# jwscook/DistributedHouseholderQR.jl

Hardware: AMD Instinct MI355X
Metric: QR GFLOP/s (F = 2mn^2 - 2/3 n^3), ||A-QR||/||A|| alongside (higher is better)
Workload: dtype f64; 1 GPU; 32768x32768 Float64 dense QR, blocked nb=128 (BASELINE configs[2]); m=32768, n=32768, nb=128, parallelism=single GPU

## Files before the change

### distributedhouseholderqr.jl_amd/csrc/dhqr_api.hip

```cpp
#include <chrono>
#include <mutex>

#include "dhqr_internal.h"
#include "dhqr_complex.h"
#include "dhqr_gemm.h"
#include "dhqr_pack.h"
#include "dhqr_panel.h"
#include "dhqr_recon.h"
#include "dhqr_solve.h"
#include "dhqr_qtb.h"
#include "dhqr_small.h"
#include "dhqr_tsqr.h"

static thread_local char g_err[512] = "";
int32_t set_err(int32_t code, const char *fmt, ...) {
  va_list ap;
  va_start(ap, fmt);
  vsnprintf(g_err, sizeof(g_err), fmt, ap);
  va_end(ap);
  return code;
}
int32_t ensure(dhqr_ctx *c, Buf &b, size_t need) {
  if (need <= b.cap) return DHQR_OK;
  if (b.p) {
// ... 478 lines not shown
    double *out = (l == lv.L()) ? Rroot : bufs[l & 1];
    hipLaunchKernelGGL(k_tsqr_node, dim3((unsigned)lv.cnt[l]), dim3(1024), 0, c->stream, (const double *)nullptr, (int64_t)0,
                       (int64_t)0, in, (int)lv.cnt[l - 1], out, Ybase ? Ybase + (size_t)lv.yoff[l] * 2 * TSQR_NN : nullptr,
                       (int64_t)0);
    in = out;
  }
  LAUNCHCHECK();
  return DHQR_OK;
}
static int32_t tsqr_pairs_down(dhqr_ctx *c, int64_t count, const double *Ybase, const double *Croot, double *ping,
                               double *pong, const double **Cleaf) {
  if (count <= 1) {
    if (Croot == nullptr) {
      hipLaunchKernelGGL(k_tsqr_identity, dim3((unsigned)(TSQR_NN / 256)), dim3(256), 0, c->stream, ping);
      LAUNCHCHECK();
      *Cleaf = ping;
    } else {
      *Cleaf = Croot;
    }
    return DHQR_OK;
  }
  const TsqrLevels lv(count);
  const double *in = Croot;
  double *bufs[2] = {ping, pong};
  for (int l = lv.L(); l >= 1; --l) {
    double *out = bufs[l & 1];
    hipLaunchKernelGGL(k_tsqr_apply, dim3((unsigned)lv.cnt[l]), dim3(1024), 0, c->stream, in,
                       Ybase + (size_t)lv.yoff[l] * 2 * TSQR_NN, (int64_t)0, 0, (int)lv.cnt[l - 1], out, (double *)nullptr,
                       (int64_t)0);
    in = out;
  }
  LAUNCHCHECK();
  *Cleaf = in;
  return DHQR_OK;
}
struct TsqrLocal {
  int64_t rows = 0, nleaf = 0, ldy = 0;
  double *R0 = nullptr, *ping = nullptr, *pong = nullptr, *Yl = nullptr, *Yp = nullptr;
  static size_t elems(int64_t rows) {
    const size_t nl = (size_t)std::max<int64_t>(1, (rows + TSQR_LEAF - 1) / TSQR_LEAF);
    return (3 * nl + 2) * TSQR_NN + nl * 2 * TSQR_NN + (size_t)TsqrLevels::node_blocks((int64_t)nl) * 2 * TSQR_NN;
  }
  void place(double *base, int64_t rows_) {
    rows = rows_;
    nleaf = std::max<int64_t>(1, (rows + TSQR_LEAF - 1) / TSQR_LEAF);
    ldy = nleaf * TSQR_LEAF;
    R0 = base;
    ping = R0 + (size_t)nleaf * TSQR_NN;
    pong = ping + (size_t)(nleaf + 1) * TSQR_NN;
    Yl = pong + (size_t)(nleaf + 1) * TSQR_NN;
    Yp = Yl + (size_t)nleaf * 2 * TSQR_NN;
  }
};
static int32_t tsqr_local_up(dhqr_ctx *c, const TsqrLocal &t, const double *P, int64_t ldp, double *Rroot, bool keep) {
  if (t.rows <= 0) {
    HIPCHECK(hipMemsetAsync(Rroot, 0, TSQR_NN * sizeof(double), c->stream));
    if (keep) HIPCHECK(hipMemsetAsync(t.Yl, 0, (size_t)t.nleaf * 2 * TSQR_NN * sizeof(double), c->stream));
    return DHQR_OK;
  }
  double *lvl0 = (t.nleaf == 1) ? Rroot : t.R0;
  hipLaunchKernelGGL(k_tsqr_node, dim3((unsigned)t.nleaf), dim3(1024), 0, c->stream, P, ldp, t.rows, (const double *)nullptr, 0,
                     lvl0, keep ? t.Yl : (double *)nullptr, t.ldy);
  LAUNCHCHECK();
  if (t.nleaf == 1) return DHQR_OK;
  return tsqr_pairs_up(c, lvl0, t.nleaf, Rroot, keep ? t.Yp : nullptr, t.ping, t.pong);
}
static int32_t tsqr_local_down(dhqr_ctx *c, const TsqrLocal &t, const double *Croot) {
  if (t.rows <= 0) return DHQR_OK;
  const double *Cleaf = nullptr;
  CHECK(tsqr_pairs_down(c, t.nleaf, t.Yp, Croot, t.ping, t.pong, &Cleaf));
  hipLaunchKernelGGL(k_tsqr_apply, dim3((unsigned)t.nleaf), dim3(1024), 0, c->stream, Cleaf, (const double *)t.Yl, t.ldy, 1, 0,
                     (double *)nullptr, t.Yl, t.ldy);
  LAUNCHCHECK();
  return DHQR_OK;
}
static int32_t tsqr_local_r(dhqr_ctx *c, const double *P, int64_t ldp, int64_t rows, double *Rout) {
  CHECK(ensure(c, c->tsq, TsqrLocal::elems(rows)));
  TsqrLocal t;
  t.place(c->tsq.p, rows);
  return tsqr_local_up(c, t, P, ldp, Rout, false);
}

static inline size_t panel_rbuf_elems() { return 6 * (size_t)DHQR_NBV * DHQR_NBV + 1024; }
static inline double *panel_rbuf(dhqr_ctx *c, int panel_idx) { return c->rbuf.p + (size_t)(panel_idx & 1) * panel_rbuf_elems(); }
static int32_t panel_commit_enqueue(dhqr_ctx *c, hipStream_t stream, double *P, int64_t rows, int64_t ldp, double *alpha,
                                    const PanelBuf &pb, int panel_idx, int part = 0) {
  const size_t NN = (size_t)DHQR_NBV * DHQR_NBV;
  const double *Rref = panel_rbuf(c, panel_idx) + 3 * NN, *altmp = panel_rbuf(c, panel_idx) + 6 * NN;
  if (part == 1) {
    hipLaunchKernelGGL(k_commit_alpha, dim3(1), dim3(DHQR_NBV), 0, stream, altmp, (int)DHQR_NBV, (double *)nullptr, pb.alpha,
                       (const int *)c->dstat, panel_idx);
  } else {
    dim3 grid((unsigned)std::min<int64_t>((rows + 255) / 256, 64), DHQR_NBV);
    hipLaunchKernelGGL(k_commit_panel, grid, dim3(256), 0, stream, P, ldp, rows, (const double *)pb.V, pb.ldv, Rref, altmp, alpha,
                       part == 2 ? (double *)nullptr : pb.alpha, (const int *)c->dstat, panel_idx);
  }
  LAUNCHCHECK();
  return DHQR_OK;
}
static int32_t panel_fast_enqueue(dhqr_ctx *c, double *P, int64_t rows, int64_t ldp, double *alpha, const PanelBuf &pb,
                                  int passes, int panel_idx, hipEvent_t ev_v = nullptr, hipEvent_t ev_t = nullptr) {
  const int64_t ldv = pb.ldv;
  const size_t NN = (size_t)DHQR_NBV * DHQR_NBV;
  CHECK(ensure(c, c->rbuf, 2 * panel_rbuf_elems()));
  if (passes == 2) CHECK(ensure(c, c->vts, (size_t)panel_elems(rows)));
  if (passes == 3) CHECK(ensure(c, c->tsq, TsqrLocal::elems(rows)));
  CHECK(ensure(c, c->sfull, NN));
  if (c->ev_commit[panel_idx & 1]) HIPCHECK(hipStreamWaitEvent(c->stream, c->ev_commit[panel_idx & 1], 0));
  double *R1 = panel_rbuf(c, panel_idx), *negR1inv = R1 + NN, *Rf = R1 + 2 * NN, *Rref = R1 + 3 * NN, *negMinv = R1 + 4 * NN;
  double *G = R1 + 5 * NN, *altmp = R1 + 6 * NN;
  int *bflag = c->dstat + 1;
  CHECK(prof_begin(c, CAT_PANEL));
  const bool was = c->profiling;
  c->profiling = false;
  auto body = [&]() -> int32_t {
    const double *X = P;
    int64_t ldx = ldp;
    if (passes == 3) {
      TsqrLocal t;
      t.place(c->tsq.p, rows);
      CHECK(tsqr_local_up(c, t, P, ldp, Rf, true));
      CHECK(tsqr_local_down(c, t, nullptr));
      hipLaunchKernelGGL(k_tsqr_identity, dim3((unsigned)(NN / 256)), dim3(256), 0, c->stream, R1);
      X = t.Yl;
      ldx = t.ldy;
      launch_recon_top(c, X, ldx, R1, G, Rref, negMinv);
      hipLaunchKernelGGL(k_tsqr_sign_cols, dim3((unsigned)(NN / 256)), dim3(256), 0, c->stream, negMinv, (const double *)Rf);
    } else if (passes == 2) {
      CHECK(gram128(c, P, ldp, rows, G));
      double *Q1 = c->vts.p;
      const int64_t ldq = panel_ldv(rows);
      launch_chol_inv(c, G, nullptr, R1, negR1inv, bflag);
      CHECK(mul128(c, P, ldp, rows, negR1inv, Q1, ldq));
      CHECK(gram128(c, Q1, ldq, rows, G));
      launch_chol_inv(c, G, R1, Rf, nullptr, bflag);
      launch_recon_top(c, P, ldp, Rf, altmp, Rref, negMinv);
    } else {
      CHECK(gram128(c, P, ldp, rows, G));
      hipLaunchKernelGGL((k_panel_top<false>), dim3(1), dim3(1024), 0, c->stream, (const double *)G, (const double *)P, ldp, altmp,
                         Rref, negMinv, bflag);
    }
    if (c->fuse_fix) {
      CHECK(mul128(c, X, ldx, rows, negMinv, pb.V, ldv, passes == 3 ? G : altmp));
    } else {
      CHECK(mul128(c, X, ldx, rows, negMinv, pb.V, ldv));
      hipLaunchKernelGGL(k_recon_fix, dim3(NN / 256), dim3(256), 0, c->stream, pb.V, ldv,
                         (const double *)(passes == 3 ? G : altmp), (const double *)negMinv);
    }
    if (ev_v) HIPCHECK(hipEventRecord(ev_v, c->stream));
    if (passes == 3)
      hipLaunchKernelGGL(k_tsqr_final_r, dim3(NN / 256), dim3(256), 0, c->stream, (const double *)Rf, (const double *)G, Rref,
                         altmp);
    CHECK(gram128(c, pb.V, ldv, rows, c->sfull.p));
    hipLaunchKernelGGL(k_build_t, dim3(1), dim3(1024), 0, c->stream, (const double *)c->sfull.p, (int)DHQR_NBV, pb.T, pb.Tt,
                       c->recon_tol, c->dstat, panel_idx, pb.alpha + DHQR_NBV, c->tt_keep);
    if (ev_t) HIPCHECK(hipEventRecord(ev_t, c->stream));
    else CHECK(panel_commit_enqueue(c, c->stream, P, rows, ldp, alpha, pb, panel_idx));
    LAUNCHCHECK();
    return DHQR_OK;
  };
  const int32_t rc = body();
  c->profiling = was;
  CHECK(rc);
  if (c->profiling)
    for (int64_t j = 0; j + 1 < DHQR_NBV; ++j) c->st.bytes_panel += 16.0 * (double)(rows - j) * (double)(DHQR_NBV - j - 1);
  CHECK(prof_end(c));
  return DHQR_OK;
}
static inline bool panel_fast_eligible(dhqr_ctx *c, int64_t rows, int64_t w) {
  return c->panel_impl == 3 && w == DHQR_NBV && rows >= 2 * DHQR_NBV;
}

static int32_t factor_panel_sync(dhqr_ctx *c, double *P, int64_t rows, int64_t w, int64_t ldp, double *alpha,
                                 const PanelBuf &pb) {
  if (panel_fast_eligible(c, rows, w)) {
    const int last_rung = std::max(c->cholqr_passes, c->tsqr_rung == 1 ? 3 : 2);
    for (int passes = c->cholqr_passes; passes <= last_rung; ++passes) {
      CHECK(status_reset(c));
      CHECK(panel_fast_enqueue(c, P, rows, ldp, alpha, pb, passes, 0));
      int failed = 0;
      CHECK(status_read(c, &failed));
      if (failed == INT_MAX) {
        c->n_fast++;
        if (passes == 3) c->n_tsqr++;
        return DHQR_OK;
      }
    }
    CHECK(status_reset(c));
    c->n_fallback++;
  }
  if (c->panel_impl >= 2 && !(c->partial_unblocked && rows > 256 && rows <= c->partial_unblocked_max_rows))
    return factor_panel_v2(c, P, rows, w, ldp, alpha, pb);
  CHECK(factor_unblocked_cols(c, P, rows, w, ldp, alpha, CAT_PANEL));
  return panel_pack_and_t(c, P, rows, w, ldp, alpha, pb);
}

static int32_t comm_allreduce_sum(dhqr_comm *cm, double *dbuf, int64_t count, hipStream_t stream);

static inline int64_t nn_row_chunks(const dhqr_ctx *c, int64_t row_tiles) {
  if (c->nn_split <= 1 || c->cur_ws != 0) return 1;
  return std::max<int64_t>(1, std::min<int64_t>(c->nn_split, row_tiles / c->nn_chunk_tiles));
}

static int32_t narrow_vtc(dhqr_ctx *c, const double *Vp, int64_t ldv, int64_t rows, const double *C, int64_t ldc,
                          int64_t ncols, bool vec, Buf &part, double *Y) {
  const int64_t ntiles = (ncols + 127) / 128, ld2 = 2 * DHQR_NBV, wstride = ld2 * ncols;
  int64_t nsplit, rps;
  pick_split(rows, 2 * ntiles, 512, 256 / ntiles, &nsplit, &rps, 512, 64);
  CHECK(ensure(c, part, (size_t)nsplit * (size_t)wstride));
  const dim3 grid((unsigned)ntiles, (unsigned)nsplit, 2);
  if (vec)
    hipLaunchKernelGGL((k_gemm_tn<2, 1, 128>), grid, dim3(256), 0, c->stream, Vp, ldv, C, ldc, 1, (int64_t)0, rows, ncols, rps, part.p,
                       ld2, wstride);
  else
    hipLaunchKernelGGL((k_gemm_tn<1, 1, 128>), grid, dim3(256), 0, c->stream, Vp, ldv, C, ldc, 1, (int64_t)0, rows, ncols, rps, part.p,
                       ld2, wstride);
  hipLaunchKernelGGL(k_reduce_splits, dim3((unsigned)((wstride + 63) / 64)), dim3(256), 0, c->stream, (const double *)part.p, (int)nsplit,
                     wstride, wstride, Y);
  return DHQR_OK;
}

static int32_t pair_vtc(dhqr_ctx *c, const double *Vp, int64_t ldv, int64_t rows, const double *C, int64_t ldc,
                        int64_t ncols, bool vec, double *Y) {
  const int64_t ntiles = (ncols + 127) / 128;
  if (ntiles <= 2) return narrow_vtc(c, Vp, ldv, rows, C, ldc, ncols, vec, c->ws[c->cur_ws].w1, Y);
  int64_t nsplit, rps;
  const int64_t slots = wide_slots(c, ncols);
  pick_split(rows, ntiles, slots, ntiles <= 2 ? 256 : 64, &nsplit, &rps, slots, ntiles <= 2 ? 64 : 128);
  if (ntiles >= c->tn_model_min_tiles) {
    const int64_t cap = std::min<int64_t>(64, std::max<int64_t>(1, rows / 512));
    double best = 1e300;
    int64_t bns = 1;
    for (int64_t ns = 1; ns <= cap; ++ns) {
      if (ns > 1 && ntiles * ns > 3072) break;
      int64_t r = (rows + ns - 1) / ns;
      r = (r + G_KT - 1) / G_KT * G_KT;
      const int64_t rounds = (ntiles * ns + slots - 1) / slots;
      const double est = (double)rounds * (double)r + (double)ns * (double)ncols * 4.79e-3 + 40.0 * (double)rounds;
      if (est < best) { best = est; bns = ns; }
    }
    int64_t r = (rows + bns - 1) / bns;
    r = (r + G_KT - 1) / G_KT * G_KT;
    rps = r;
    nsplit = std::max<int64_t>(1, (rows + r - 1) / r);
  }
  dhqr_ctx::WS &ws = c->ws[c->cur_ws];
  const int64_t ld2 = 2 * DHQR_NBV, wstride = ld2 * ncols;
  if (ntiles >= c->tn_model_min_tiles && ntiles <= 1024 && rows >= 1024) {
    const int64_t FU = 128, S = (rows + FU - 1) / FU, U = ntiles * S;
    const int64_t G = std::min<int64_t>(U, slots), q = (U + G - 1) / G, Gq = (U + q - 1) / q;
    int R = c->tn2_rgroups;
    if (R == 0) R = rows >= c->tn2_rg8_rows ? 8 : rows >= c->tn2_rg4_rows ? 4 : rows >= c->tn2_rg2_rows ? 2 : 1;
    if (G < 64 || S < 4 * R) R = 1;
    if (R > 1) {
      int P = 0;
      for (int g = 0; g < R; ++g) P = std::max(P, tn2_sk_pieces(tn2_sk_group_of(g, R, G, S, ntiles, q)));
      CHECK(ensure(c, ws.w1, (size_t)R * (size_t)P * (size_t)wstride));
      if (vec)
        hipLaunchKernelGGL((k_gemm_tn2<2, true>), dim3((unsigned)G), dim3(512), 0, c->stream, Vp, ldv, C, ldc, rows, ncols, FU, ws.w1.p, wstride, q, R, P);
      else
        hipLaunchKernelGGL((k_gemm_tn2<1, true>), dim3((unsigned)G), dim3(512), 0, c->stream, Vp, ldv, C, ldc, rows, ncols, FU, ws.w1.p, wstride, q, R, P);
      hipLaunchKernelGGL(k_reduce_pieces, dim3((unsigned)((wstride + 255) / 256)), dim3(256), 0, c->stream, (const double *)ws.w1.p, S, q,
                         wstride, wstride, Y, R, P, G, ntiles);
      return DHQR_OK;
    }
    const int64_t pieces = (q >= S) ? 2 : (S + q - 1) / q + 1;
    CHECK(ensure(c, ws.w1, (size_t)pieces * (size_t)wstride));
    if (vec)
      hipLaunchKernelGGL((k_gemm_tn2<2, true>), dim3((unsigned)Gq), dim3(512), 0, c->stream, Vp, ldv, C, ldc, rows, ncols, FU, ws.w1.p, wstride, q, 1, 0);
    else
      hipLaunchKernelGGL((k_gemm_tn2<1, true>), dim3((unsigned)Gq), dim3(512), 0, c->stream, Vp, ldv, C, ldc, rows, ncols, FU, ws.w1.p, wstride, q, 1, 0);
    hipLaunchKernelGGL(k_reduce_pieces, dim3((unsigned)((wstride + 255) / 256)), dim3(256), 0, c->stream, (const double *)ws.w1.p, S, q,
                       wstride, wstride, Y, 1, 0, Gq, ntiles);
    return DHQR_OK;
  }
  CHECK(ensure(c, ws.w1, (size_t)nsplit * (size_t)wstride));
  const dim3 gtn((unsigned)std::min<int64_t>(ntiles * nsplit, slots)), gred((unsigned)((wstride + 63) / 64));
  if (vec)
    hipLaunchKernelGGL((k_gemm_tn2<2>), gtn, dim3(512), 0, c->stream, Vp, ldv, C, ldc, rows, ncols, rps, ws.w1.p, wstride, (int64_t)0, 1, 0);
  else
    hipLaunchKernelGGL((k_gemm_tn2<1>), gtn, dim3(512), 0, c->stream, Vp, ldv, C, ldc, rows, ncols, rps, ws.w1.p, wstride, (int64_t)0, 1, 0);
  hipLaunchKernelGGL(k_reduce_splits, gred, dim3(256), 0, c->stream, (const double *)ws.w1.p, (int)nsplit, wstride, wstride, Y);
  return DHQR_OK;
}

static int32_t pair_tw(dhqr_ctx *c, double *Y, const double *Ta, const double *Tb, const double *Sba, double *W,
                       int64_t ldw, int64_t ncols) {
  const int64_t ntiles = (ncols + 127) / 128, ld2 = 2 * DHQR_NBV;
  double *Ya = Y, *Yb = Y + DHQR_NBV;
  if (ntiles <= 2) {
    const int64_t NN_ = (int64_t)DHQR_NBV * DHQR_NBV;
    hipLaunchKernelGGL((k_tw_fused<true>), dim3((unsigned)((ncols + 3) / 4)), dim3(256), 0, c->stream, (const double *)Y, ncols,
                       Ta + NN_, Tb + NN_, Sba, W, ldw);
    return DHQR_OK;
  }
  hipLaunchKernelGGL((k_gemm_tn<2, 1, 128>), dim3((unsigned)ntiles, 1), dim3(256), 0, c->stream, Ta, (int64_t)DHQR_NBV,
                     (const double *)Ya, ld2, 1, (int64_t)0, (int64_t)DHQR_NBV, ncols, (int64_t)DHQR_NBV, W, ldw, (int64_t)0);
  launch_nn_sub<128>(c, true, dim3(1, (unsigned)ntiles), Sba, (int64_t)DHQR_NBV, (const double *)W, ldw, Yb, ld2,
                     (int64_t)DHQR_NBV, ncols, 0, false);
  hipLaunchKernelGGL((k_gemm_tn<2, 1, 128>), dim3((unsigned)ntiles, 1), dim3(256), 0, c->stream, Tb, (int64_t)DHQR_NBV,
                     (const double *)Yb, ld2, 1, (int64_t)0, (int64_t)DHQR_NBV, ncols, (int64_t)DHQR_NBV, W + DHQR_NBV, ldw,
                     (int64_t)0);
  return DHQR_OK;
}

static int32_t pair_apply(dhqr_ctx *c, const double *Vp, int64_t ldv, int64_t rows, const double *Ta,
                          const double *Tb, const double *Sba, double *C, int64_t ncols, int64_t ldc,
                          dhqr_comm *ar = nullptr, int64_t rows_b_in = -1) {
// ... 225 lines not shown
  for (int64_t j = 0; j < n; ++j) memcpy(dst + j * ldd, src + j * lds, (size_t)m * sizeof(double));
}

struct DeviceGuard {
  int prev = -1;
  ~DeviceGuard() {
    if (prev >= 0) (void)hipSetDevice(prev);
  }
};
static int32_t enter_ctx(dhqr_ctx *c, DeviceGuard &g) {
  if (!c) return set_err(DHQR_EINVAL, "null context");
  int cur = -1;
  HIPCHECK(hipGetDevice(&cur));
  if (cur != c->device) {
    HIPCHECK(hipSetDevice(c->device));
    g.prev = cur;
  }
  return DHQR_OK;
}
#define ENTER(c_)   \
  DeviceGuard dg_; \
  CHECK(enter_ctx(c_, dg_))
static inline bool no_columns(int64_t m, int64_t n) { return n == 0 && m >= 0; }

static int32_t check_mat(const void *A, int64_t m, int64_t n, int64_t lda, bool need_tall) {
  if (!A) return set_err(DHQR_EINVAL, "null matrix pointer");
  if (m <= 0 || n <= 0) return set_err(DHQR_EINVAL, "m and n must be positive (m=%lld n=%lld)", (long long)m, (long long)n);
  if (need_tall && m < n) return set_err(DHQR_EINVAL, "m >= n required (m=%lld n=%lld)", (long long)m, (long long)n);
  if (lda < m) return set_err(DHQR_EINVAL, "leading dimension %lld < m=%lld", (long long)lda, (long long)m);
  if (lda > (int64_t)0xFFFFFFFFLL / 128)
    return set_err(DHQR_EINVAL, "leading dimension %lld too large (128 * ld must stay below 2^32 elements)", (long long)lda);
  return DHQR_OK;
}

static int32_t apply_q_impl(dhqr_ctx *c, const double *dA, int64_t m, int64_t n, int64_t lda,
                            const double *dalpha, double *dB, int64_t nrhs, int64_t ldb, int trans,
                            bool triangular) {
  const int64_t npan = (n + DHQR_NBV - 1) / DHQR_NBV;
  CHECK(ensure(c, c->vt, (size_t)panel_elems(m)));
  for (int64_t q = 0; q < npan; ++q) {
    const int64_t k = trans ? q : npan - 1 - q;
    const int64_t c0 = k * DHQR_NBV, w = std::min<int64_t>(DHQR_NBV, n - c0), rows = m - c0;
    const double *P = dA + c0 + c0 * lda;
    const PanelBuf pb = vt_view(c->vt.p, rows);
    CHECK(panel_pack_and_t(c, P, rows, w, lda, dalpha ? dalpha + c0 : nullptr, pb));
    if (triangular) {
      if (nrhs - c0 > 0) CHECK(panel_apply(c, pb, rows, dB + c0 + c0 * ldb, nrhs - c0, ldb, trans));
    } else {
      CHECK(panel_apply(c, pb, rows, dB + c0, nrhs, ldb, trans));
    }
  }
  return DHQR_OK;
}

extern "C" {

int32_t dhqr_version(void) { return DHQR_VERSION; }
const char *dhqr_last_error(void) { return g_err; }

int32_t dhqr_device_count(int32_t *count) {
  if (!count) return set_err(DHQR_EINVAL, "null count");
  int n = 0;
  hipError_t e = hipGetDeviceCount(&n);
  if (e != hipSuccess) {
    *count = 0;
    return set_err(DHQR_ENODEVICE, "hipGetDeviceCount: %s", hipGetErrorString(e));
  }
  *count = n;
  return DHQR_OK;
}

int32_t dhqr_create(dhqr_ctx **out, int32_t device) {
  if (!out) return set_err(DHQR_EINVAL, "null ctx out-pointer");
  *out = nullptr;
  int n = 0;
  hipError_t e = hipGetDeviceCount(&n);
  if (e != hipSuccess || n <= 0)
    return set_err(DHQR_ENODEVICE, "no HIP device visible (%s); libdhqr has no CPU fallback",
                   e != hipSuccess ? hipGetErrorString(e) : "count = 0");
  if (device < 0 || device >= n) return set_err(DHQR_EINVAL, "device %d out of range [0,%d)", device, n);
  HIPCHECK(hipSetDevice(device));
  hipDeviceProp_t prop;
  HIPCHECK(hipGetDeviceProperties(&prop, device));
  if (strncmp(prop.gcnArchName, "gfx950", 6) != 0)
    return set_err(DHQR_ENODEVICE, "device %d is %s; this library is built for gfx950 only", device,
                   prop.gcnArchName);
  dhqr_ctx *c = new dhqr_ctx();
  c->device = device;
  c->coop = prop.cooperativeLaunch != 0;
  g_live_ctx[device & 63].fetch_add(1);
  memset(&c->st, 0, sizeof(c->st));
  auto init = [&]() -> int32_t {
    HIPCHECK(hipStreamCreateWithFlags(&c->own, hipStreamNonBlocking));
    c->stream = c->own;
    {
      int lo = 0, hi = 0;
      HIPCHECK(hipDeviceGetStreamPriorityRange(&lo, &hi));
      HIPCHECK(hipStreamCreateWithPriority(&c->hi, hipStreamNonBlocking, hi));
      if (const char *e = getenv("DHQR_LANE_SIDE")) c->lane_side = atoi(e) != 0;
      c->hi_priority = hi;
    }
    if (const char *e = getenv("DHQR_LOOKAHEAD")) c->lookahead = atoi(e) != 0;
    {
      int ncu = 0;
      if (hipDeviceGetAttribute(&ncu, hipDeviceAttributeMultiprocessorCount, device) == hipSuccess && ncu > 0) {
        c->rankk_wgs = ncu;
        c->ncu = ncu;
      }
    }
    if (const char *e = getenv("DHQR_SPARE_CUS")) {
      c->spare_cus = std::max(0, std::min(c->ncu - 8, atoi(e)));
      c->spare_cus_set = true;
    }
    if (const char *e = getenv("DHQR_QUAD")) c->quad = atoi(e) != 0;
    if (const char *e = getenv("DHQR_QUAD_MIN_COLS")) c->quad_min_cols = std::max<int64_t>(0, atoll(e));
    { long long v; if (tune_get("rankk_wgs", &v)) c->rankk_wgs = std::max(2, (int)v); }
    if (const char *e = getenv("DHQR_RANKK")) c->rankk = c->rankk_tall = c->rankk_xtall = std::min(5, std::max(1, atoi(e)));
    if (const char *e = getenv("DHQR_RANKK_MAX")) c->rankk_max = std::min(DHQR_RK_KMAX, std::max(1, atoi(e)));
    { long long v; if (tune_get("rankk_max_min_cols", &v)) c->rankk_max_min_cols = std::max(0, (int)v); }
    { long long v; if (tune_get("nn_chunk_tiles", &v)) c->nn_chunk_tiles = std::max(1, (int)v); }
    if (const char *e = getenv("DHQR_NN_SPLIT")) c->nn_split = std::min(16, std::max(1, atoi(e)));
    if (const char *e = getenv("DHQR_RANKK_PIPE")) c->rankk_pipe = std::min(2, std::max(0, atoi(e)));
    { long long v; if (tune_get("tn_min_tiles", &v)) c->tn_model_min_tiles = (int)v; }
    { long long v; if (tune_get("small_flags", &v)) c->small_flags = v != 0; }
    { long long v; if (tune_get("short_panel_small", &v)) c->short_panel_small = v != 0; }
    { long long v; if (tune_get("partial_unblocked", &v)) c->partial_unblocked = v != 0; }
    { long long v; if (tune_get("partial_unblocked_max_rows", &v)) c->partial_unblocked_max_rows = v; }
    { long long v; if (tune_get("small_spin_limit", &v)) c->small_spin_limit = (int)v; }
    { long long v; if (tune_get("tn2_rgroups", &v)) c->tn2_rgroups = (int)v; }
    { long long v; if (tune_get("tn2_rg8_rows", &v)) c->tn2_rg8_rows = v; }
    { long long v; if (tune_get("tn2_rg4_rows", &v)) c->tn2_rg4_rows = v; }
    { long long v; if (tune_get("tn2_rg2_rows", &v)) c->tn2_rg2_rows = v; }
    { long long v; if (tune_get("tn_spare", &v)) c->tn_spare = std::max(0, std::min((c->ncu - 8) / 2, (int)v)); }
    { long long v; if (tune_get("tn_spare_cols", &v)) c->tn_spare_cols = v; }
    if (const char *e = getenv("DHQR_PAIR")) c->pair = atoi(e) != 0;
    if (const char *e = getenv("DHQR_PAIR_MIN_N")) c->pair_min_n = atoll(e);
    HIPCHECK(hipHostMalloc((void **)&c->hflag, 4 * sizeof(int), hipHostMallocDefault));
    HIPCHECK(hipMalloc((void **)&c->dstat, 16 * sizeof(int)));
    HIPCHECK(hipMalloc((void **)&c->zflags, DHQR_PIPE_INTS * sizeof(int)));
    HIPCHECK(hipMemsetAsync(c->zflags, 0, DHQR_PIPE_INTS * sizeof(int), c->stream));
    {
      int limit = DHQR_PIPE_SPIN_LIMIT;
      { long long v; if (tune_get("spin_limit", &v)) limit = std::max(1, (int)v); }
      HIPCHECK(hipMemcpyAsync(c->zflags + DHQR_PIPE_LIMIT_OFFSET, &limit, sizeof(int), hipMemcpyHostToDevice, c->stream));
      HIPCHECK(hipStreamSynchronize(c->stream));
    }
    if (const char *e = getenv("DHQR_SMALL")) c->small_route = atoi(e) != 0;
    if (const char *e = getenv("DHQR_ZPIPE")) c->zpipe = atoi(e) != 0;
    if (const char *e = getenv("DHQR_SOLVE_PIPE")) c->solve_pipe = std::max(0, std::min(3, atoi(e)));
    if (const char *e = getenv("DHQR_KEEP_T")) c->keep_t = atoi(e) != 0;
    { long long v; if (tune_get("qtb_vec", &v)) c->qtb_vec = (int)v; }
    { long long v; if (tune_get("gram_strips", &v)) c->gram_strips = v != 0; }
    { long long v; if (tune_get("fuse_fix", &v)) c->fuse_fix = v != 0; }
    { long long v; if (tune_get("commit_off", &v)) c->commit_off = (int)v; }
    hipLaunchKernelGGL(k_set_status, dim3(1), dim3(64), 0, c->stream, c->dstat, INT_MAX);
    LAUNCHCHECK();
    HIPCHECK(hipStreamSynchronize(c->stream));
    return DHQR_OK;
  };
  const int32_t rc_init = init();
  if (rc_init != DHQR_OK) {
    (void)dhqr_destroy(c);
    return rc_init;
  }
  if (const char *e = getenv("DHQR_CHOLQR_PASSES")) c->cholqr_passes = atoi(e) == 2 ? 2 : 1;
  if (const char *e = getenv("DHQR_TSQR")) {
    if (atoi(e) != 0) c->cholqr_passes = 3;
  }
  if (const char *e = getenv("DHQR_TSQR_RUNG")) c->tsqr_rung = atoi(e) != 0 ? 1 : 0;
  if (const char *e = getenv("DHQR_PANEL")) {
    const int v = atoi(e);
    if (v >= 1 && v <= 3) c->panel_impl = v;
  }
  *out = c;
  return DHQR_OK;
}

int32_t dhqr_destroy(dhqr_ctx *c) {
  if (!c) return DHQR_OK;
  g_live_ctx[c->device & 63].fetch_sub(1);
  (void)hipSetDevice(c->device);
  (void)hipStreamSynchronize(c->stream);
  (void)hipDeviceSynchronize();
  cs_state_free(c);
  rs_state_free(c);
  if (c->hio) {
    hio_free(*c->hio);
    delete c->hio;
    c->hio = nullptr;
  }
  Buf *bufs[] = {&c->vbuf, &c->vt, &c->vts, &c->ws[0].w1, &c->ws[0].w1r, &c->ws[0].w2, &c->ws[1].w1,
                 &c->ws[1].w1r, &c->ws[1].w2, &c->ws[2].w1, &c->ws[2].w1r, &c->ws[2].w2, &c->spart, &c->spart2, &c->sfull, &c->scratch, &c->pbuf, &c->rbuf, &c->tsq, &c->zsolve_lo, &c->host_mat, &c->sv_T, &c->sv_S, &c->sv_part, &c->sv_small, &c->tc_T, &c->tc_alpha, &c->small_dev, &c->sv_bkp};
  for (Buf *b : bufs)
    if (b->p) (void)hipFree(b->p);
  for (auto &e : c->evs) {
    (void)hipEventDestroy(e.a);
    (void)hipEventDestroy(e.b);
  }
  if (c->hflag) (void)hipHostFree(c->hflag);
  if (c->small_pin) (void)hipHostFree(c->small_pin);
  if (c->dstat) (void)hipFree(c->dstat);
  if (c->zflags) (void)hipFree(c->zflags);
  for (hipEvent_t e : c->zev)
    if (e) (void)hipEventDestroy(e);
  if (c->hi) (void)hipStreamDestroy(c->hi);
  if (c->hi2) (void)hipStreamDestroy(c->hi2);
  if (c->cstream) (void)hipStreamDestroy(c->cstream);
  for (hipEvent_t e : c->ev_commit)
    if (e) (void)hipEventDestroy(e);
  if (c->own) (void)hipStreamDestroy(c->own);
  delete c;
  return DHQR_OK;
}

int32_t dhqr_set_stream(dhqr_ctx *c, void *s) {
  ENTER(c);
  c->stream = (hipStream_t)s;
  return DHQR_OK;
}
int32_t dhqr_use_own_stream(dhqr_ctx *c) {
  ENTER(c);
  c->stream = c->own;
  return DHQR_OK;
}
static int32_t pipe_error_report(dhqr_ctx *c, int e) {
  HIPCHECK(hipMemsetAsync(c->zflags + DHQR_PIPE_ERR_OFFSET, 0, sizeof(int), c->stream));
  HIPCHECK(hipStreamSynchronize(c->stream));
  return set_err(DHQR_EHIP, "an inter-workgroup pipeline (k_zpanel_pipe / rankk_lead_pipe / k_backsub_pipe, launch %d) gave up "
                 "waiting for a lower-indexed workgroup: the results of that call are invalid; DHQR_ZPIPE=0 / DHQR_RANKK_PIPE=0 / "
                 "DHQR_SOLVE_PIPE=0 select the kernels without inter-workgroup waits", e);
}
static int32_t pipe_error_check(dhqr_ctx *c) {
  if (!c->zflags) return DHQR_OK;
  int e = 0;
  HIPCHECK(hipMemcpy(&e, c->zflags + DHQR_PIPE_ERR_OFFSET, sizeof(int), hipMemcpyDeviceToHost));
  if (e == 0) return DHQR_OK;
  if (e == 0x7ffffffe && c->retry.valid) {
    const dhqr_ctx::SolveRetry r = c->retry;
    c->retry.valid = false;
    HIPCHECK(hipMemsetAsync(c->zflags + DHQR_PIPE_ERR_OFFSET, 0, sizeof(int), c->stream));
    HIPCHECK(hipMemcpyAsync(r.b, c->sv_bkp.p, (size_t)r.m * sizeof(double), hipMemcpyDeviceToDevice, c->stream));
    const bool was = c->profiling;
    c->profiling = false;
    const int32_t rc = solve_pipelined(c, r.A, r.m, r.n, r.lda, r.alpha, r.b, false);
    c->profiling = was;
    CHECK(rc);
    HIPCHECK(hipStreamSynchronize(c->stream));
    c->n_solve_retry++;
    HIPCHECK(hipMemcpy(&e, c->zflags + DHQR_PIPE_ERR_OFFSET, sizeof(int), hipMemcpyDeviceToHost));
    if (e == 0) return DHQR_OK;
  }
  return pipe_error_report(c, e);
}

int32_t dhqr_synchronize(dhqr_ctx *c) {
  ENTER(c);
  HIPCHECK(hipStreamSynchronize(c->stream));
  return pipe_error_check(c);
}
int32_t dhqr_trim(dhqr_ctx *c) {
  ENTER(c);
  HIPCHECK(hipStreamSynchronize(c->stream));
  HIPCHECK(hipDeviceSynchronize());
  Buf *bs[] = {&c->host_mat, &c->sv_T, &c->sv_S, &c->sv_part, &c->sv_small, &c->tc_T, &c->tc_alpha, &c->vts, &c->tsq, &c->zsolve_lo,
               &c->small_dev, &c->sv_bkp};
  c->retry.valid = false;
  if (c->small_pin) {
    (void)hipHostFree(c->small_pin);
    c->small_pin = nullptr;
    c->small_pin_cap = 0;
  }
  for (Buf *b : bs)
    if (b->p) {
      (void)hipFree(b->p);
      b->p = nullptr;
      b->cap = 0;
    }
  c->tc_valid = false;
  c->sv_units_dev = nullptr;
  if (c->cs)
    for (Buf &b : c->cs->gbuf)
      if (b.p) {
        (void)hipFree(b.p);
        b.p = nullptr;
        b.cap = 0;
      }
  if (c->hio) {
    hio_free(*c->hio);
    delete c->hio;
    c->hio = nullptr;
  }
  return pipe_error_check(c);
}
int32_t dhqr_set_profiling(dhqr_ctx *c, int32_t on) {
  ENTER(c);
  if (c->profiling && !on) CHECK(prof_resolve(c));
  c->profiling = on != 0;
  return DHQR_OK;
}
int32_t dhqr_reset_stats(dhqr_ctx *c) {
  ENTER(c);
  HIPCHECK(hipStreamSynchronize(c->stream));
  c->ev_used = 0;
  memset(&c->st, 0, sizeof(c->st));
  c->n_fast = c->n_fallback = 0;
  c->n_tsqr = 0;
// ... 1853 lines not shown
```

### distributedhouseholderqr.jl_amd/csrc/dhqr_internal.h

```cpp
#pragma once
#include <hip/hip_runtime.h>

#include <algorithm>
#include <atomic>
#include <climits>
#include <chrono>
#include <cmath>
#include <cstdarg>
#include <cstdio>
#include <cstring>
#include <vector>

#include "../../include/dhqr.h"
#include "dhqr_common.h"

int32_t set_err(int32_t code, const char *fmt, ...);
#define HIPCHECK(expr)                                                                        \
  do {                                                                                        \
    hipError_t e_ = (expr);                                                                   \
    if (e_ != hipSuccess)                                                                     \
      return set_err(DHQR_EHIP, "%s failed: %s (%s:%d)", #expr, hipGetErrorString(e_),        \
                     __FILE__, __LINE__);                                                     \
  } while (0)
#define CHECK(expr)                  \
  do {                               \
    int32_t rc_ = (expr);            \
    if (rc_ != DHQR_OK) return rc_;  \
  } while (0)
#define LAUNCHCHECK() HIPCHECK(hipGetLastError())

enum { CAT_PANEL = 0, CAT_TBUILD, CAT_VTA, CAT_TW, CAT_AVW, CAT_RANK1, CAT_SOLVE, CAT_N };

struct Buf {
  double *p = nullptr;
  size_t cap = 0;
};

struct dhqr_ctx {
  int device = 0;
  hipStream_t own = nullptr, stream = nullptr;
  bool profiling = false;
  hipStream_t hi = nullptr;
  hipStream_t hi2 = nullptr;
  int lane_side = 1;
  int hi_priority = 0;
  int tn_spare = 32;
  int64_t tn_spare_cols = 16384;
  int tn_model_min_tiles = 32;
  int rankk_wgs = 256;
  int rankk = 5;
  int nn_chunk_tiles = 48;
  int nn_split = 4;
  int rankk_pipe = 1;
  int rankk_max_min_cols = 4096;
  int rankk_unfit = 0;
  int rankk_max = 8;
  int rankk_xtall = 5;
  int rankk_tall = 5;
  int ncu = 256;
  int spare_cus = 0;
  bool spare_cus_set = false;
  int quad = 1;
  int64_t quad_min_cols = 10240;
  struct WS { Buf w1, w1r, w2; } ws[3];
  int cur_ws = 0;
  bool lookahead = true;
  Buf vbuf, vt, vts, spart, spart2, sfull, scratch, pbuf;
  Buf zsolve_lo;
  Buf sv_T, sv_S, sv_part, sv_small;
  std::vector<int> sv_units;
  int64_t sv_m = -1, sv_n = -1, sv_rps = 0;
  const int *sv_units_dev = nullptr;
  Buf tc_T, tc_alpha;
  double *tt_keep = nullptr, *tc_base = nullptr;
  const double *tc_A = nullptr;
  int64_t tc_m = 0, tc_n = 0, tc_lda = 0;
  bool tc_valid = false;
  int keep_t = 1;
  int solve_pipe = 1;
  int qtb_vec = -1;
  struct SolveRetry {
    bool valid = false;
    const double *A = nullptr, *alpha = nullptr;
    double *b = nullptr;
    int64_t m = 0, n = 0, lda = 0;
  } retry;
  Buf sv_bkp;
  int64_t n_solve_retry = 0;
  int gram_strips = 1;
  int small_spin_limit = 1 << 20;
  int partial_unblocked = 1;
  int64_t partial_unblocked_max_rows = 4608;
  int short_panel_small = 1;
  int small_flags = 1;
  int tn2_rgroups = 1;
  int64_t tn2_rg8_rows = 20480, tn2_rg4_rows = 10240, tn2_rg2_rows = 5120;
  int fuse_fix = 1;
  int commit_off = -1;
  hipStream_t cstream = nullptr;
  hipEvent_t ev_commit[2] = {nullptr, nullptr};
  int small_route = 1;
  double *small_pin = nullptr;
  size_t small_pin_cap = 0;
  Buf small_dev;
  unsigned long long small_epoch = 0;
  bool coop = false;
  Buf host_mat;
  int pair = 1;
  int64_t pair_min_n = 4096;
  int panel_impl = 3;
  int zpipe = 1;
  hipEvent_t zev[5] = {nullptr, nullptr, nullptr, nullptr, nullptr};
  int *zflags = nullptr;
  int zepoch = 0;
  int *hflag = nullptr;
  int *dstat = nullptr;
  int epoch = -1;
  Buf rbuf;
  Buf tsq;
  int tsqr_rung = -1;
  int n_tsqr = 0;
  int64_t n_fast = 0, n_fallback = 0;
  int cholqr_passes = 1;
  double recon_tol = 2e-12;
  int ib = 64;
  struct CsState *cs = nullptr;
  struct RsState *rs = nullptr;
  int32_t (*panel_hook)(void *, int64_t, hipEvent_t) = nullptr;
  void *panel_hook_arg = nullptr;
  struct HostIo *hio = nullptr;
  int64_t n_resume = 0;
  struct Ev { hipEvent_t a, b; int cat; int start_from = -1; };
  std::vector<Ev> evs;
  size_t ev_used = 0;
  dhqr_stats st;
};


int32_t ensure(dhqr_ctx *c, Buf &b, size_t need);
bool tune_get(const char *key, long long *out);
static inline bool aligned16(const void *p) { return (((uintptr_t)p) & 15) == 0; }
int32_t prof_begin(dhqr_ctx *c, int cat);
int32_t prof_end(dhqr_ctx *c);
int32_t prof_switch(dhqr_ctx *c, int cat);
#define DHQR_RK_KMAX 8
int32_t factor_unblocked_cols(dhqr_ctx *c, double *P, int64_t rows, int64_t ncols, int64_t ldp, double *alpha, int cat);
```

### distributedhouseholderqr.jl_amd/csrc/dhqr_recon.h

```cpp
#pragma once
#include "dhqr_common.h"

#define RC_N 128

__device__ __forceinline__ void rc_upper_inverse_regs(const double (&r)[4][4], double (&x)[4][4],
                                                       double *dinv, double *rowbuf2, double *colbuf2) {
  const int t = threadIdx.x, ti = t >> 5, tk = t & 31;
  double acc[4][4];
#pragma unroll
  for (int a = 0; a < 4; ++a) {
    if (ti == tk) dinv[ti + 32 * a] = 1.0 / r[a][a];
#pragma unroll
    for (int b = 0; b < 4; ++b) { acc[a][b] = 0.0; x[a][b] = 0.0; }
  }
  __syncthreads();
#pragma unroll
  for (int la = 3; la >= 0; --la)
    for (int lm = 31; lm >= 0; --lm) {
      const int l = la * 32 + lm;
      double *rowbuf = rowbuf2 + (l & 1) * RC_N, *colbuf = colbuf2 + (l & 1) * RC_N;
      if (ti == lm) {
        const double di = dinv[l];
#pragma unroll
        for (int b = 0; b < 4; ++b) {
// ... 332 lines not shown
#pragma unroll
  for (int x = 0; x < 4; ++x)
#pragma unroll
    for (int y = 0; y < 4; ++y) negMinv[(ti + 32 * x) + (tk + 32 * y) * RC_N] = mm[x][y];
  __syncthreads();
  double x12[4];
  rc_upper_inverse_blocked(negMinv, RC_N, false, L, x12);
  __syncthreads();
  rc5_emit(L, x12, [&](int i, int k, double v) { negMinv[i + k * RC_N] = -v; });
}

__device__ unsigned long long g_top_phase[8];
template <bool TIME = false>
__device__ __forceinline__ void rc_chol_replay_invert(double (&g)[4][4], double (&a)[4][4], double *rbuf, double *wrow,
                                                      double *vcol, rc5_lds &L, double *__restrict__ alpha,
                                                      double *__restrict__ Rref, double *__restrict__ negMinv,
                                                      int *__restrict__ flag) {
  const int t = threadIdx.x, ti = t >> 5, tk = t & 31, lane = t & 63;
  double *qu = &L.T1[0][0];
#pragma unroll
  for (int ja = 0; ja < 4; ++ja)
    for (int jm = 0; jm < 32; ++jm) {
      const int j = ja * 32 + jm;
      const int src = (lane & 32) + jm;
      long long tq0 = 0, tq1 = 0, tq2 = 0, tq3 = 0;
      if constexpr (TIME) tq0 = clock64();
      double d = __shfl(g[ja][ja], src, 64);
      const double ajj = __shfl(a[ja][ja], src, 64);
      if constexpr (TIME) {
        asm volatile("" : "+v"(d));
        tq1 = clock64();
      }
      double *rb = rbuf + (j & 1) * RC_N, *wr = wrow + (j & 1) * RC_N, *vc = vcol + (j & 1) * RC_N;
      if (ti == jm) {
        if (!(d > 0.0)) {
          if (tk == 0) flag[0] = 1;
          d = 1.0;
        }
        double r, rinv;
        dhqr_sqrt_rsqrt(d, r, rinv);
        const double al = r * dhqr_alphafactor(ajj);
        const double u = dhqr_rcp(ajj - al);
        if (tk == 0) {
          qu[j] = r * (r + fabs(ajj));
          qu[RC_N + j] = u;
        }
        const double sg = (al == 0.0) ? 0.0 : (al < 0.0 ? -1.0 : 1.0);
#pragma unroll
        for (int y = 0; y < 4; ++y) {
          const int k = tk + 32 * y;
          const double x = (k == j) ? r : g[ja][y] * rinv;
          g[ja][y] = x;
          rb[k] = (k > j) ? x : 0.0;
          const double rr = sg * x;
          const double dl = (k > j) ? (a[ja][y] - rr) : 0.0;
          wr[k] = dl * u;
          negMinv[j + k * RC_N] = dl;
          Rref[j + k * RC_N] = (k > j) ? rr : 0.0;
        }
        if (tk == 0) alpha[j] = al;
      }
      if (tk == jm) {
#pragma unroll
        for (int x = 0; x < 4; ++x) {
          const int i = ti + 32 * x;
          vc[i] = (i > j) ? a[x][ja] : 0.0;
        }
      }
      if constexpr (TIME) tq2 = clock64();
      __syncthreads();
      if constexpr (TIME) tq3 = clock64();
#pragma unroll
      for (int x = 0; x < 4; ++x) {
        if (x < ja) continue;
        const double ri = rb[ti + 32 * x], vi = vc[ti + 32 * x];
#pragma unroll
        for (int y = 0; y < 4; ++y) {
          if (y < ja) continue;
          const double rk = rb[tk + 32 * y];
          if (y >= x) g[x][y] = fma(-ri, rk, g[x][y]);
          a[x][y] = fma(-vi, wr[tk + 32 * y], a[x][y]);
        }
      }
      if constexpr (TIME) {
        asm volatile("" : "+v"(a[3][3]), "+v"(g[3][3]));
        const long long tq4 = clock64();
        if (t == 0) {
          g_top_phase[0] += (unsigned long long)(tq1 - tq0);
          g_top_phase[1] += (unsigned long long)(tq2 - tq1);
          g_top_phase[2] += (unsigned long long)(tq3 - tq2);
          g_top_phase[3] += (unsigned long long)(tq4 - tq3);
          g_top_phase[5] += 1ull;
        }
      }
    }
  long long tinv = 0;
  if constexpr (TIME) tinv = clock64();
  __syncthreads();
  if (t < RC_N) {
    const double sq = sqrt(qu[t]);
    qu[t] = sq * qu[RC_N + t];
    qu[RC_N + t] = sq;
  }
  __syncthreads();
  double x12[4];
  rc_upper_inverse_blocked(negMinv, RC_N, false, L, x12, qu);
  __syncthreads();
  rc5_emit(L, x12, [&](int i, int k, double v) { negMinv[i + k * RC_N] = -v; });
  if constexpr (TIME) {
    __builtin_amdgcn_s_waitcnt(0);
    if (t == 0) g_top_phase[4] += (unsigned long long)(clock64() - tinv);
  }
}

__global__ __launch_bounds__(1024) void k_recon_top(const double *__restrict__ P, int64_t ldp,
                                                     const double *__restrict__ R,
                                                     double *__restrict__ alpha,
                                                     double *__restrict__ Rref,
                                                     double *__restrict__ negMinv) {
  __shared__ double wrow[2 * RC_N], vcol[2 * RC_N];
  __shared__ rc5_lds L;
  const int t = threadIdx.x, ti = t >> 5, tk = t & 31;
  double a[4][4], r[4][4];
#pragma unroll
  for (int x = 0; x < 4; ++x)
#pragma unroll
    for (int y = 0; y < 4; ++y) {
      const int i = ti + 32 * x, k = tk + 32 * y;
      a[x][y] = P[i + (int64_t)k * ldp];
      r[x][y] = R[i + k * RC_N];
    }
  rc_replay_and_invert(a, r, wrow, vcol, L, alpha, Rref, negMinv);
}

template <bool TIME = false>
__global__ __launch_bounds__(1024) void k_panel_top(const double *__restrict__ G, const double *__restrict__ P,
                                                     int64_t ldp, double *__restrict__ alpha,
                                                     double *__restrict__ Rref, double *__restrict__ negMinv,
                                                     int *__restrict__ flag) {
  __shared__ double rbuf[2 * RC_N], wrow[2 * RC_N], vcol[2 * RC_N];
  __shared__ rc5_lds L;
  const int t = threadIdx.x, ti = t >> 5, tk = t & 31;
  double g[4][4], a[4][4];
#pragma unroll
  for (int x = 0; x < 4; ++x)
#pragma unroll
    for (int y = 0; y < 4; ++y) {
      g[x][y] = G[(ti + 32 * x) + (tk + 32 * y) * RC_N];
      a[x][y] = P[(ti + 32 * x) + (int64_t)(tk + 32 * y) * ldp];
    }
  rc_chol_replay_invert<TIME>(g, a, rbuf, wrow, vcol, L, alpha, Rref, negMinv, flag);
}

__global__ __launch_bounds__(256) void k_recon_fix(double *__restrict__ Vw, int64_t ldv,
                                                   const double *__restrict__ alpha,
                                                   const double *__restrict__ negMinv) {
  const int idx = blockIdx.x * blockDim.x + threadIdx.x;
  if (idx >= RC_N * RC_N) return;
  const int i = idx & (RC_N - 1), j = idx >> 7;
  double x = 0.0;
  if (i >= j) x = Vw[i + (int64_t)j * ldv] + alpha[i] * negMinv[i + j * RC_N];
  Vw[i + (int64_t)j * ldv] = x;
}

__global__ void k_adopt_status(const double *__restrict__ statword, int *__restrict__ stat) {
  if (threadIdx.x == 0 && blockIdx.x == 0) {
    const double w = *statword;
    if (w < (double)stat[0]) stat[0] = (int)w;
  }
}
__global__ __launch_bounds__(128) void k_commit_alpha(const double *__restrict__ src, int w, double *__restrict__ dst1,
                                                      double *__restrict__ dst2, const int *__restrict__ stat,
                                                      int epoch) {
  if (stat != nullptr && stat[0] <= epoch) return;
  const int j = threadIdx.x;
  const double a = (j < w) ? src[j] : 0.0;
  if (dst1 && j < w) dst1[j] = a;
  if (dst2) dst2[j] = a;
}
__global__ __launch_bounds__(128) void k_zero_rows(double *__restrict__ X, int64_t ldx, int nrows) {
  for (int r = threadIdx.x; r < nrows; r += blockDim.x) X[r + (int64_t)blockIdx.x * ldx] = 0.0;
}

__global__ __launch_bounds__(256) void k_recon_write_r(double *__restrict__ P, int64_t ldp,
                                                       const double *__restrict__ Rref,
                                                       const int *__restrict__ stat, int epoch) {
  if (stat != nullptr && stat[0] <= epoch) return;
  const int idx = blockIdx.x * blockDim.x + threadIdx.x;
  if (idx >= RC_N * RC_N) return;
  const int i = idx & (RC_N - 1), j = idx >> 7;
  if (i < j) P[i + (int64_t)j * ldp] = Rref[idx];
}
__global__ __launch_bounds__(256) void k_commit_panel(double *__restrict__ P, int64_t ldp, int64_t rows,
                                                      const double *__restrict__ Vw, int64_t ldv,
                                                      const double *__restrict__ Rref, const double *alpha_src,
                                                      double *alpha_dst1, double *alpha_dst2,
                                                      const int *__restrict__ stat, int epoch) {
  if (stat != nullptr && stat[0] <= epoch) return;
  const int64_t p = blockIdx.y;
  const int64_t stride = (int64_t)gridDim.x * blockDim.x;
  for (int64_t r = p + (int64_t)blockIdx.x * blockDim.x + threadIdx.x; r < rows; r += stride) P[r + p * ldp] = Vw[r + p * ldv];
  if (blockIdx.x == 0) {
    for (int64_t r = threadIdx.x; r < p; r += blockDim.x) P[r + p * ldp] = Rref[r + p * RC_N];
    if (threadIdx.x == 0) {
      const double a = alpha_src[p];
      if (alpha_dst1) alpha_dst1[p] = a;
      if (alpha_dst2) alpha_dst2[p] = a;
    }
  }
}
__global__ void k_set_statword(const int *__restrict__ stat, double *__restrict__ statword) {
  if (threadIdx.x == 0 && blockIdx.x == 0) *statword = (double)stat[0];
}
__global__ void k_axpy1(double *__restrict__ x, const double *__restrict__ s, int n) {
  const int i = threadIdx.x;
  if (i < n) x[i] += s[i];
}
```

Baseline: 59920 GFLOP/s.

## Add slot-based MFMA triangular inverse kernel for building the T factor

Adds a new single-workgroup kernel, k_build_t_slot, that forms the compact-WY T factor. It inverts the 128x128 unit upper triangle using small per-thread triangular solves on the diagonal blocks and f64 MFMA 16x16x4 products for the off-diagonal blocks, staging data in dynamic LDS. The kernel is enabled by default through a new lane_slot tunable and replaces the older k_build_t launch. The aim is a shorter serial panel critical path per block column. In exchange it uses a large LDS allocation and a waves-per-eu hint, and the numerics of the inverse change.

```diff
diff --git a/distributedhouseholderqr.jl_amd/csrc/dhqr_api.hip b/distributedhouseholderqr.jl_amd/csrc/dhqr_api.hip
--- a/distributedhouseholderqr.jl_amd/csrc/dhqr_api.hip
+++ b/distributedhouseholderqr.jl_amd/csrc/dhqr_api.hip
@@ -654,8 +654,18 @@
       hipLaunchKernelGGL(k_tsqr_final_r, dim3(NN / 256), dim3(256), 0, c->stream, (const double *)Rf, (const double *)G, Rref,
                          altmp);
     CHECK(gram128(c, pb.V, ldv, rows, c->sfull.p));
-    hipLaunchKernelGGL(k_build_t, dim3(1), dim3(1024), 0, c->stream, (const double *)c->sfull.p, (int)DHQR_NBV, pb.T, pb.Tt,
-                       c->recon_tol, c->dstat, panel_idx, pb.alpha + DHQR_NBV, c->tt_keep);
+    if (c->lane_slot) {
+#ifdef __HIPCC__
+      static const hipError_t attr = hipFuncSetAttribute(reinterpret_cast<const void *>(&k_build_t_slot),
+                                                         hipFuncAttributeMaxDynamicSharedMemorySize, (int)sizeof(rc_buildt_slot_lds));
+      HIPCHECK(attr);
+#endif
+      hipLaunchKernelGGL(k_build_t_slot, dim3(1), dim3(1024), sizeof(rc_buildt_slot_lds), c->stream, (const double *)c->sfull.p,
+                         (int)DHQR_NBV, pb.T, pb.Tt, c->recon_tol, c->dstat, panel_idx, pb.alpha + DHQR_NBV, c->tt_keep);
+    } else {
+      hipLaunchKernelGGL(k_build_t, dim3(1), dim3(1024), 0, c->stream, (const double *)c->sfull.p, (int)DHQR_NBV, pb.T, pb.Tt,
+                         c->recon_tol, c->dstat, panel_idx, pb.alpha + DHQR_NBV, c->tt_keep);
+    }
     if (ev_t) HIPCHECK(hipEventRecord(ev_t, c->stream));
     else CHECK(panel_commit_enqueue(c, c->stream, P, rows, ldp, alpha, pb, panel_idx));
     LAUNCHCHECK();
@@ -1187,6 +1197,7 @@
     { long long v; if (tune_get("qtb_vec", &v)) c->qtb_vec = (int)v; }
     { long long v; if (tune_get("gram_strips", &v)) c->gram_strips = v != 0; }
     { long long v; if (tune_get("fuse_fix", &v)) c->fuse_fix = v != 0; }
+    { long long v; if (tune_get("lane_slot", &v)) c->lane_slot = v != 0; }
     { long long v; if (tune_get("commit_off", &v)) c->commit_off = (int)v; }
     hipLaunchKernelGGL(k_set_status, dim3(1), dim3(64), 0, c->stream, c->dstat, INT_MAX);
     LAUNCHCHECK();
diff --git a/distributedhouseholderqr.jl_amd/csrc/dhqr_internal.h b/distributedhouseholderqr.jl_amd/csrc/dhqr_internal.h
--- a/distributedhouseholderqr.jl_amd/csrc/dhqr_internal.h
+++ b/distributedhouseholderqr.jl_amd/csrc/dhqr_internal.h
@@ -96,6 +96,7 @@
   int tn2_rgroups = 1;
   int64_t tn2_rg8_rows = 20480, tn2_rg4_rows = 10240, tn2_rg2_rows = 5120;
   int fuse_fix = 1;
+  int lane_slot = 1;
   int commit_off = -1;
   hipStream_t cstream = nullptr;
   hipEvent_t ev_commit[2] = {nullptr, nullptr};
diff --git a/distributedhouseholderqr.jl_amd/csrc/dhqr_recon.h b/distributedhouseholderqr.jl_amd/csrc/dhqr_recon.h
--- a/distributedhouseholderqr.jl_amd/csrc/dhqr_recon.h
+++ b/distributedhouseholderqr.jl_amd/csrc/dhqr_recon.h
@@ -508,6 +508,175 @@
   rc_chol_replay_invert<TIME>(g, a, rbuf, wrow, vcol, L, alpha, Rref, negMinv, flag);
 }
 
+struct rc5s_lds {
+  double W[4 * 32 * RC5_LDD];
+  double X[2][3][32][RC5_LDD];
+  double dinv[RC_N];
+};
+__device__ __forceinline__ double &rc5s_x(rc5s_lds &L, int h, int r, int c) {
+  return L.X[h][(r >> 5) + (c >> 5)][r & 31][c & 31];
+}
+__device__ __forceinline__ double rc5s_xr(const rc5s_lds &L, int h, int r, int c) {
+  const double v = L.X[h][(r >> 5) + (c >> 5)][r & 31][c & 31];
+  return (r >= 32 && c < 32) ? 0.0 : v;
+}
+__device__ __forceinline__ void rc_upper_inverse_slot(const double *__restrict__ Mg, int ncols, bool unit, rc5s_lds &L,
+                                                      double (&x12)[4], const double *rs = nullptr) {
+  const int t = threadIdx.x;
+  double *Ud = L.W;
+  for (int e = t; e < 2 * 3 * 32 * RC5_LDD; e += 1024) (&L.X[0][0][0][0])[e] = 0.0;
+#pragma unroll
+  for (int r = 0; r < 4; ++r) {
+    const int e = t + 1024 * r, d = e >> 10, i = e & 31, l = (e >> 5) & 31;
+    Ud[(32 * d + i) * RC5_LDD + l] = rc5_in(Mg, 32 * d + i, 32 * d + l, ncols, rs);
+  }
+  if (t < RC_N) L.dinv[t] = unit ? 1.0 : 1.0 / (rs ? rs[RC_N + t] : Mg[t + t * RC_N]);
+  __syncthreads();
+  if (t < RC_N) {
+    const int d = t >> 5, hb = (t >> 4) & 1, k = t & 15, q = 16 * hb;
+    double x[16];
+#pragma unroll
+    for (int i = 15; i >= 0; --i) {
+      double s = 0.0;
+#pragma unroll
+      for (int l = i + 1; l < 16; ++l) s = fma(Ud[(32 * d + q + i) * RC5_LDD + q + l], x[l], s);
+      x[i] = (i == k) ? L.dinv[32 * d + q + k] : ((i < k) ? -s * L.dinv[32 * d + q + i] : 0.0);
+    }
+    double(&Xd)[32][RC5_LDD] = L.X[d >> 1][2 * (d & 1)];
+#pragma unroll
+    for (int i = 0; i < 16; ++i) Xd[q + i][q + k] = x[i];
+  }
+  __syncthreads();
+  if (t < 256) {
+    const int d = t >> 6, ln = t & 63, pi = ln & 15, pk = ln >> 4;
+    double(&Xd)[32][RC5_LDD] = L.X[d >> 1][2 * (d & 1)];
+    dhqr_d4 tb = (dhqr_d4){0.0, 0.0, 0.0, 0.0};
+#pragma unroll
+    for (int ks = 0; ks < 4; ++ks)
+      tb = __builtin_amdgcn_mfma_f64_16x16x4f64(Ud[(32 * d + pi) * RC5_LDD + 16 + 4 * ks + pk], Xd[16 + 4 * ks + pk][16 + pi], tb, 0, 0, 0);
+    dhqr_d4 xb = (dhqr_d4){0.0, 0.0, 0.0, 0.0};
+#pragma unroll
+    for (int ks = 0; ks < 4; ++ks) xb = __builtin_amdgcn_mfma_f64_16x16x4f64(Xd[pi][4 * ks + pk], tb[ks], xb, 0, 0, 0);
+#pragma unroll
+    for (int g = 0; g < 4; ++g) Xd[pk + 4 * g][16 + pi] = -xb[g];
+  }
+  __syncthreads();
+  double b3[4];
+#pragma unroll
+  for (int r = 0; r < 4; ++r) {
+    const int e = t + 1024 * r;
+    b3[r] = rc5_in(Mg, e & 63, 64 + (e >> 6), ncols, rs);
+  }
+  {
+    const int i = t & 31, l = t >> 5;
+    Ud[i * RC5_LDD + l] = rc5_in(Mg, i, 32 + l, ncols, rs);
+    Ud[(32 + i) * RC5_LDD + l] = rc5_in(Mg, 64 + i, 96 + l, ncols, rs);
+  }
+  __syncthreads();
+  const int lane = t & 63, w = t >> 6, fi = lane & 15, fk = lane >> 4;
+  {
+    double *T1 = Ud + 64 * RC5_LDD;
+    const int h = w >> 2, ti = (w >> 1) & 1, tj = w & 1;
+    if (w < 8) {
+      dhqr_d4 acc = (dhqr_d4){0.0, 0.0, 0.0, 0.0};
+#pragma unroll
+      for (int ks = 0; ks < 8; ++ks)
+        acc = __builtin_amdgcn_mfma_f64_16x16x4f64(Ud[(32 * h + 16 * ti + fi) * RC5_LDD + 4 * ks + fk],
+                                                  rc5s_x(L, h, 32 + 4 * ks + fk, 32 + 16 * tj + fi), acc, 0, 0, 0);
+#pragma unroll
+      for (int g = 0; g < 4; ++g) T1[(32 * h + 16 * ti + fk + 4 * g) * RC5_LDD + 16 * tj + fi] = acc[g];
+    }
+    __syncthreads();
+    if (w < 8) {
+      dhqr_d4 acc = (dhqr_d4){0.0, 0.0, 0.0, 0.0};
+#pragma unroll
+      for (int ks = 0; ks < 8; ++ks)
+        acc = __builtin_amdgcn_mfma_f64_16x16x4f64(rc5s_x(L, h, 16 * ti + fi, 4 * ks + fk),
+                                                  T1[(32 * h + 4 * ks + fk) * RC5_LDD + 16 * tj + fi], acc, 0, 0, 0);
+#pragma unroll
+      for (int g = 0; g < 4; ++g) rc5s_x(L, h, 16 * ti + fk + 4 * g, 32 + 16 * tj + fi) = -acc[g];
+    }
+  }
+  __syncthreads();
+#pragma unroll
+  for (int r = 0; r < 4; ++r) {
+    const int e = t + 1024 * r;
+    L.W[(e & 63) * RC5_LDH + (e >> 6)] = b3[r];
+  }
+  __syncthreads();
+  {
+    const int ti = w & 3, tj = w >> 2;
+    dhqr_d4 acc = (dhqr_d4){0.0, 0.0, 0.0, 0.0};
+#pragma unroll
+    for (int ks = 0; ks < 16; ++ks)
+      acc = __builtin_amdgcn_mfma_f64_16x16x4f64(L.W[(16 * ti + fi) * RC5_LDH + 4 * ks + fk], rc5s_xr(L, 1, 4 * ks + fk, 16 * tj + fi),
+                                                acc, 0, 0, 0);
+    __syncthreads();
+#pragma unroll
+    for (int g = 0; g < 4; ++g) L.W[(16 * ti + fk + 4 * g) * RC5_LDH + 16 * tj + fi] = acc[g];
+    __syncthreads();
+    acc = (dhqr_d4){0.0, 0.0, 0.0, 0.0};
+#pragma unroll
+    for (int ks = 0; ks < 16; ++ks)
+      acc = __builtin_amdgcn_mfma_f64_16x16x4f64(rc5s_xr(L, 0, 16 * ti + fi, 4 * ks + fk), L.W[(4 * ks + fk) * RC5_LDH + 16 * tj + fi],
+                                                acc, 0, 0, 0);
+#pragma unroll
+    for (int g = 0; g < 4; ++g) x12[g] = -acc[g];
+  }
+}
+template <typename F>
+__device__ __forceinline__ void rc5s_emit(const rc5s_lds &L, const double (&x12)[4], F &&put) {
+  const int t = threadIdx.x;
+#pragma unroll
+  for (int r = 0; r < 4; ++r) {
+    const int e = t + 1024 * r, i = e & 63, j = e >> 6;
+    put(i, j, rc5s_xr(L, 0, i, j));
+    put(64 + i, 64 + j, rc5s_xr(L, 1, i, j));
+    put(16 * ((t >> 6) & 3) + ((t & 63) >> 4) + 4 * r, 64 + 16 * (t >> 8) + (t & 15), x12[r]);
+    put(64 + i, j, 0.0);
+  }
+}
+
+#ifdef __HIPCC__
+#define DHQR_SLOT_LDS(T, name) extern __shared__ T name[]
+#define DHQR_SLOT_VGPR64 __attribute__((amdgpu_waves_per_eu(8)))
+#else
+#define DHQR_SLOT_LDS(T, name) __shared__ T name[1]
+#define DHQR_SLOT_VGPR64
+#endif
+struct rc_buildt_slot_lds {
+  rc5s_lds inv;
+  int bad[RC_N];
+};
+__global__ __launch_bounds__(1024) DHQR_SLOT_VGPR64 void k_build_t_slot(
+    const double *__restrict__ S, int ncols, double *__restrict__ Tout, double *__restrict__ Ttout, double tol,
+    int *__restrict__ stat, int panel_idx, double *__restrict__ statword, double *__restrict__ Tt2) {
+  DHQR_SLOT_LDS(rc_buildt_slot_lds, Ls);
+  rc5s_lds &L = Ls[0].inv;
+  int *bad = Ls[0].bad;
+  if (stat != nullptr) {
+    const int j = threadIdx.x;
+    if (j < RC_N) bad[j] = (fabs(S[j + j * RC_N] - 2.0) <= tol) ? 0 : 1;
+    __syncthreads();
+    if (j == 0) {
+      int any = stat[1];
+      for (int q = 0; q < RC_N; ++q) any |= bad[q];
+      if (any && stat[0] > panel_idx) stat[0] = panel_idx;
+      stat[1] = 0;
+      if (statword) *statword = (double)stat[0];
+    }
+  }
+  double x12[4];
+  rc_upper_inverse_slot(S, ncols, true, L, x12);
+  rc5s_emit(L, x12, [&](int i, int k, double v) {
+    Tout[i + k * RC_N] = v;
+    Ttout[k + i * RC_N] = v;
+    if (Tt2) Tt2[k + i * RC_N] = v;
+  });
+}
+
+static_assert(sizeof(rc_buildt_slot_lds) <= 90 * 1024, "lane slot: LDS budget");
+
 __global__ __launch_bounds__(256) void k_recon_fix(double *__restrict__ Vw, int64_t ldv,
                                                    const double *__restrict__ alpha,
                                                    const double *__restrict__ negMinv) {
```

Result: no change. 60100 GFLOP/s, median of 6 (+0.3%).
